# nellogrb/MultigridAnisotropicDiffusion

Measured on AMD Instinct MI355X. Metric: Mvoxel-smooths/s (and V-cycles/s) at 512^3 fp32; achieved HBM GB/s vs peak, higher is better.
Workload: dtype f32

## Files before the change

include/mad.h:

```cpp
#ifndef MAD_H
#define MAD_H

#include <stddef.h>
#include <stdint.h>

#ifdef __cplusplus
extern "C" {
#endif

#define MAD_ABI_VERSION 1

typedef enum mad_status {
  MAD_OK = 0,
  MAD_ERR_INVALID = 1,
  MAD_ERR_STATE = 2,
  MAD_ERR_DEVICE = 3,
  MAD_ERR_COMM = 4,
  MAD_ERR_SINGULAR = 5,
  MAD_ERR_UNSUPPORTED = 6,
  MAD_ERR_NOMEM = 7,
  MAD_ERR_NUMERIC = 8,
  MAD_ERR_NOT_CONVERGED = 9
} mad_status;

// ... 55 lines not shown
  uint32_t options;
  int32_t min_slab_planes;
  int32_t min_slab_voxels;
  int32_t coarse_dense_max;
  int32_t coarse_block_unknowns;
  int32_t reserved[3];
} mad_desc;

#define MAD_OPT_EAGER_RANK_VCYCLE 1u
#define MAD_OPT_OVERLAP_RANK_SWEEP 2u
#define MAD_OPT_PEER_HALO 4u
#define MAD_OPT_COARSE_NO_CHAIN 8u
#define MAD_OPT_BENCHMARK_TRACE 16u
#define MAD_OPT_NO_PLACEMENT_TUNE 32u
#define MAD_OPT_NO_RECORD_B 64u

typedef struct mad_stats {
  uint32_t steps;
  uint32_t total_cycles;
  uint32_t last_cycles;
  int32_t stalled;
  double last_relres;
  double setup_ms;
  double solve_ms;
  uint32_t num_levels;
  int32_t tensor_kind;
  int32_t colors;
  int32_t reserved[5];
} mad_stats;

// ... 10 lines not shown
int mad_set_tensor_device(mad_ctx *ctx, const void *dev_aos, int32_t dtype);
int mad_tensor_planes(const mad_ctx *ctx, int64_t *first_plane, int64_t *nplanes);
int mad_set_tensor_planes(mad_ctx *ctx, const void *host_aos, int32_t dtype,
                          int64_t first_plane, int64_t nplanes);

int mad_setup(mad_ctx *ctx);

int mad_run(mad_ctx *ctx, const void *host_in, int32_t in_dtype, void *host_out,
            int32_t out_dtype, mad_stats *stats);
int mad_run_device(mad_ctx *ctx, const void *dev_in, int32_t in_dtype, void *dev_out,
                   int32_t out_dtype, mad_stats *stats);
int mad_get_step_stats(const mad_ctx *ctx, uint32_t step, uint32_t *cycles, double *relres);
int mad_get_cycle_trace(const mad_ctx *ctx, uint32_t cap, uint32_t *step, double *relres,
                        double *seconds, uint32_t *count);
int mad_placement_trials(const mad_ctx *ctx, uint32_t cap, double *ms, uint32_t *count);

int mad_num_levels(const mad_ctx *ctx);
int mad_plan_level(const mad_desc *d, int32_t level, int64_t size[3], double spacing[3],
                   int32_t centering[3], int64_t *z_begin, int64_t *z_end,
                   int32_t *distributed);
int mad_level_info(const mad_ctx *ctx, int32_t level, int64_t size[3], double spacing[3],
                   int32_t centering[3]);

int mad_upload(mad_ctx *ctx, int32_t level, int32_t which, const double *host);
int mad_download(mad_ctx *ctx, int32_t level, int32_t which, double *host);
int mad_fill(mad_ctx *ctx, int32_t level, int32_t which, double value);
int mad_smooth(mad_ctx *ctx, int32_t level, uint32_t sweeps);
int mad_residual(mad_ctx *ctx, int32_t level, double *norm_out);
int mad_norm(mad_ctx *ctx, int32_t level, int32_t which, double *norm_out);
int mad_restrict(mad_ctx *ctx, int32_t level);
// ... 32 lines not shown
```

multigridanisotropicdiffusion_amd/_capi.py:

```python
import ctypes
import os

_HERE = os.path.dirname(os.path.abspath(__file__))
LIB_PATH = os.path.join(_HERE, "libmad_hip.so")

ABI_VERSION = 1

OK, ERR_INVALID, ERR_STATE, ERR_DEVICE, ERR_COMM, ERR_SINGULAR, ERR_UNSUPPORTED, ERR_NOMEM, \
    ERR_NUMERIC, ERR_NOT_CONVERGED = range(10)
VCYCLE, FMG, SMOOTHER = 0, 1, 2
GAUSS_SEIDEL, GAUSS_SEIDEL_LEX, WEIGHTED_JACOBI = 0, 1, 2
U8, I8, U16, I16, U32, I32, F32, F64 = range(8)
FP32, FP64, FP32_REFINE, PRECISION_AUTO = 0, 1, 2, 3
VED_HESSIAN_RECURSIVE, VED_HESSIAN_FIR = 0, 1
TENSOR_AUTO, TENSOR_ISOTROPIC, TENSOR_DIAGONAL, TENSOR_FULL = range(4)
X, B, R = 0, 1, 2
OPT_EAGER_RANK_VCYCLE = 1
OPT_OVERLAP_RANK_SWEEP = 2
OPT_PEER_HALO = 4
OPT_COARSE_NO_CHAIN = 8
OPT_BENCHMARK_TRACE = 16
OPT_NO_PLACEMENT_TUNE = 32
OPT_NO_RECORD_B = 64
VED_OPT_LINE_WALK = 1
CED_EED, CED_CED = 0, 1

EXPORTS = (
    "mad_desc_init", "mad_max_depth", "mad_create", "mad_destroy", "mad_last_error",
    "mad_get_desc", "mad_set_tensor", "mad_set_tensor_device", "mad_tensor_planes",
    "mad_set_tensor_planes", "mad_setup", "mad_run",
    "mad_run_device", "mad_get_step_stats", "mad_get_cycle_trace", "mad_placement_trials", "mad_num_levels", "mad_plan_level",
    "mad_level_info", "mad_upload",
    "mad_download", "mad_fill", "mad_smooth", "mad_residual", "mad_norm", "mad_restrict",
    "mad_residual_restrict",
    "mad_interpolate", "mad_prolongate_add", "mad_coarse_solve", "mad_vcycle", "mad_fmg",
    "mad_synchronize", "mad_bench_smooth", "mad_bench_launch_times", "mad_smooth_kernel_name", "mad_bench_vcycle", "mad_bench_synth_tensor",
    "mad_bench_synth_level", "mad_comm_unique_id", "mad_comm_init", "mad_comm_init_local", "mad_comm_init_solo",
    "mad_comm_init_rccl_solo",
    "mad_comm_selftest", "mad_slab_range", "mad_comm_allreduce_host", "mad_comm_version",
    "mad_ved_desc_init", "mad_ved_create", "mad_ved_destroy", "mad_ved_last_error",
    "mad_ved_run", "mad_ved_run_device", "mad_ved_comm_init", "mad_ved_comm_init_local",
    "mad_ved_comm_init_solo",
    "mad_ved_tensor", "mad_ved_hessian",
)

CED_EXPORTS = (
# ... 177 lines not shown
        "mad_max_depth": ([i32, i64p], i32),
        "mad_create": ([ctypes.POINTER(MadDesc), ctypes.POINTER(vp)], i32),
        "mad_destroy": ([vp], None),
        "mad_last_error": ([vp], ctypes.c_char_p),
        "mad_get_desc": ([vp, ctypes.POINTER(MadDesc)], i32),
        "mad_set_tensor": ([vp, vp, i32], i32),
        "mad_set_tensor_device": ([vp, vp, i32], i32),
        "mad_tensor_planes": ([vp, i64p, i64p], i32),
        "mad_set_tensor_planes": ([vp, vp, i32, ctypes.c_int64, ctypes.c_int64], i32),
        "mad_setup": ([vp], i32),
        "mad_run": ([vp, vp, i32, vp, i32, ctypes.POINTER(MadStats)], i32),
        "mad_run_device": ([vp, vp, i32, vp, i32, ctypes.POINTER(MadStats)], i32),
        "mad_get_step_stats": ([vp, u32, u32p, dp], i32),
        "mad_get_cycle_trace": ([vp, u32, u32p, dp, dp, u32p], i32),
        "mad_placement_trials": ([vp, u32, dp, u32p], i32),
        "mad_num_levels": ([vp], i32),
        "mad_plan_level": ([ctypes.POINTER(MadDesc), i32, i64p, dp, i32p, i64p, i64p, i32p], i32),
        "mad_level_info": ([vp, i32, i64p, dp, i32p], i32),
        "mad_upload": ([vp, i32, i32, dp], i32),
        "mad_download": ([vp, i32, i32, dp], i32),
        "mad_fill": ([vp, i32, i32, dbl], i32),
        "mad_smooth": ([vp, i32, u32], i32),
        "mad_residual": ([vp, i32, dp], i32),
        "mad_norm": ([vp, i32, i32, dp], i32),
        "mad_restrict": ([vp, i32], i32),
        "mad_residual_restrict": ([vp, i32, ctypes.POINTER(i32)], i32),
        "mad_interpolate": ([vp, i32], i32),
        "mad_prolongate_add": ([vp, i32], i32),
        "mad_coarse_solve": ([vp], i32),
        "mad_vcycle": ([vp], i32),
# ... 67 lines not shown
```

multigridanisotropicdiffusion_amd/csrc/mad_kernels.hpp:

```cpp
#pragma once
#include <hip/hip_runtime.h>

#include <climits>
#include <type_traits>
#include <cstdint>

namespace mad {

enum { KISO = 1, KDIAG = 2, KFULL = 3 };

template <int DIM, int KIND>
struct CoefLayout {
  static constexpr int NA = (KIND == KISO) ? 1 : DIM;
  static constexpr int NG = DIM;
  static constexpr int NE = (KIND == KFULL) ? DIM * (DIM - 1) / 2 : 0;
  static constexpr int N = NA + NG + NE;
};

inline int coef_count(int dim, int kind) {
  int na = (kind == KISO) ? 1 : dim;
  int ne = (kind == KFULL) ? dim * (dim - 1) / 2 : 0;
  return na + dim + ne;
}

// ... 868 lines not shown
    u_dst[e] = q < PL ? q : -1;
    u_src[e] = (uint32_t)(mirror(y0 - 1 + lj, ny) * sy + mirror(x0 - 1 + li, nx)) * TS;
  }
  const int i = x0 + tx, j = y0 + ty;
  const bool ok = i < nx && j < ny;
  const uint32_t rec_off = ok ? (uint32_t)(ty * sy + (tx & 1) * hx0 + (tx >> 1)) * (TS * RS) : 0u;
  const uint32_t pt_off = ok ? (uint32_t)(ty * sy + tx) * TS : 0u;
  const uint32_t pt_off_b = ok ? (uint32_t)(ty * sy + tx) * (uint32_t)sizeof(TB) : 0u;
  const int64_t rbase = (int64_t)y0 * sy + (x0 >> 1), pbase = (int64_t)y0 * sy + x0;
  const int il = (ty + 1) * RX + (tx + 1);
  constexpr int oyp = RX, oym = -RX;

  T up[UPT];
  T raw[RS];
  T bv = T(0);
  auto load_plane = [&](int m) {
    m = min(max(m, zlo), zhi - 1);
    const __amdgpu_buffer_rsrc_t rs = buf_rsrc(u + (int64_t)m * sz);
#pragma unroll
    for (int e = 0; e < UPT; ++e) up[e] = buf_load<T>(rs, u_src[e], 0u);
    if (ue) {
      const __amdgpu_buffer_rsrc_t re = buf_rsrc(ue + (int64_t)m * sz);
#pragma unroll
      for (int e = 0; e < UPT; ++e)
        up[e] = up[e] + (T)buf_load<TE>(re, (u_src[e] / TS) * (uint32_t)sizeof(TE), 0u);
    }
  };
  auto put_plane = [&](int m) {
    T* P = ring + (m & 3) * PL;
#pragma unroll
    for (int e = 0; e < UPT; ++e)
      if (e < UPT - 1 || u_dst[e] >= 0) P[u_dst[e]] = up[e];
  };
  auto load_pt = [&](int m) {
    m = min(max(m, 0), g.nz - 1);
    buf_load_rec<T, RS>(buf_rsrc(cf + ((int64_t)m * sz + rbase) * RS), rec_off, raw);
    if constexpr (!BREC) bv = (T)buf_load<TB>(buf_rsrc(b + (int64_t)m * sz + pbase), pt_off_b, 0u);
  };

  if (z0 - 1 >= zlo) {
// ... 166 lines not shown
    v += (T(1) - omega) * P0[0];
    load_pt(m + 1);
    if (ok) buf_store<T>(v, buf_rsrc(uo + (int64_t)m * sz + pbase), pt_off);
  }
}

template <typename T>
__global__ void __launch_bounds__(256) sumsq_k(const T* __restrict__ x, int64_t n,
                                               double* __restrict__ part) {
  double s = 0.0;
  for (int64_t q = blockIdx.x * (int64_t)blockDim.x + threadIdx.x; q < n;
       q += (int64_t)gridDim.x * blockDim.x) {
    const double v = (double)x[q];
    s += v * v;
  }
  s = block_sum<256>(s);
  if (threadIdx.x == 0) part[blockIdx.x] = s;
}

__global__ void __launch_bounds__(256) reduce_final_k(const double* __restrict__ part, int64_t n,
                                                      double* __restrict__ out) {
  double s = 0.0;
  for (int64_t q = threadIdx.x; q < n; q += blockDim.x) s += part[q];
  s = block_sum<256>(s);
  if (threadIdx.x == 0) out[0] = s;
}

template <typename W>
__device__ __forceinline__ void rtaps4(int I, int nc, int cell, int* idx, W* w) {
  const bool endv = !cell && (I == 0 || I == nc - 1);
// ... 833 lines not shown
```

multigridanisotropicdiffusion_amd/csrc/mad_solver.hip:

```cpp
#include <hip/hip_runtime.h>
#include <rocblas/rocblas.h>
#include <rocsolver/rocsolver.h>

#include <algorithm>
#include <chrono>
#include <cmath>
#include <cstdio>
#include <cstdlib>
#include <cstring>
#include <memory>
#include <mutex>
#include <stdexcept>
#include <string>
#include <thread>
#include <type_traits>
#include <vector>

#include "../../include/mad.h"
#include "mad_alloc.hpp"
#include "mad_coarse.hpp"
#include "mad_comm.hpp"
#include "mad_kernels.hpp"

using namespace mad;
// ... 197 lines not shown
  std::vector<double> step_relres;
  struct TracePoint {
    uint32_t step;
    double relres, seconds;
  };
  std::vector<TracePoint> trace;
  bool bench_trace() const { return (d.options & MAD_OPT_BENCHMARK_TRACE) != 0; }
  bool trace_active = false;
  uint32_t trace_step = 0;
  double trace_rhs = 1.0;
  std::chrono::steady_clock::time_point trace_t0{};
  void trace_push(double rr) {
    trace.push_back({trace_step, rr, std::chrono::duration<double>(std::chrono::steady_clock::now() - trace_t0).count()});
  }
  double setup_ms = 0.0;
  Comm comm;
  ~mad_ctx();
};

constexpr int TENSOR_GHOST = GHOST + 4;

struct SolverBase {
  virtual ~SolverBase() {}
  virtual void setup(mad_ctx* c) = 0;
  virtual void upload(int l, int which, const double* h) = 0;
  virtual void download(int l, int which, double* h) = 0;
  virtual void fill(int l, int which, double v) = 0;
  virtual void smooth(int l, unsigned n) = 0;
  virtual double residual(int l, bool want_norm) = 0;
  virtual double norm(int l, int which) = 0;
// ... 633 lines not shown
      REQUIRE(zr.nchunks >= 2 && zr.zc >= GHOST, MAD_ERR_UNSUPPORTED, "slab too thin for the single-launch sweep");
      *flip = 1;
      *sig = part == 3 ? L.sig : nullptr;
    } else if (part == 1) {
      zr = ZRange{0, boundary_planes(), nz - boundary_planes(), 2};
    } else if (part == 2) {
      const int ni = nz - 2 * boundary_planes();
      int chunks = std::max(1, std::min((fc.blocks + tiles - 1) / tiles, std::max(1, ni / 16)));
      const int zc = (ni + chunks - 1) / chunks;
      zr = ZRange{boundary_planes(), zc, zc, (ni + zc - 1) / zc};
    }
    return zr;
  }

  template <int KD, int TX, int TY, int NT>
  void launch_fused(LevelData<T>& L, const FusedCfg& fc, int part, bool zu = false) {
    const int ntx = (L.g.nx + TX - 1) / TX, nty = (L.g.ny + TY - 1) / TY;
    const int tiles = ntx * nty;
    int flip = 0;
    uint32_t* sig = nullptr;
    const ZRange zr = part_range(L, tiles, fc, part, &flip, &sig);
    const unsigned nb = (unsigned)(tiles * zr.nchunks);
    constexpr int NC = (KD == KFULL) ? 4 : 2;
    using FG = FusedGeom<NC, TX, TY>;
    constexpr size_t lds_u = sizeof(T) * FG::NP * FG::PLANE;
    REQUIRE(lds_u <= 160 * 1024, MAD_ERR_UNSUPPORTED,
            "fused GS tile needs " + std::to_string(lds_u) + " B of LDS (> 160 KiB)");
    constexpr size_t lds_bl = sizeof(T) * (FG::NP + NC) * FG::PLANE;
    constexpr bool bl_fits = lds_bl <= 160 * 1024;
    const bool bl = fused_b_lds(L);
    const size_t lds = bl ? lds_bl : lds_u;
    constexpr int MW = sizeof(T) == 8 ? 2 : 4;
    const PeerOut<T> po = part == 4 ? peer_out(L, buffer_index(L, L.t)) : PeerOut<T>{{nullptr, nullptr}, {nullptr, nullptr}};
    auto run = [&](auto kern) {
      {
        static std::mutex attr_mu;
        static std::vector<const void*> attr;
        std::lock_guard<std::mutex> lk(attr_mu);
        if (std::find(attr.begin(), attr.end(), (const void*)kern) == attr.end()) {
          HIP_CHECK(hipFuncSetAttribute((const void*)kern, hipFuncAttributeMaxDynamicSharedMemorySize,
                                        (int)lds));
          attr.push_back((const void*)kern);
        }
      }
      hipLaunchKernelGGL(kern, dim3(nb), dim3(NT), lds, c_->stream, L.x, L.t, L.bs ? L.bs : L.b, L.cf, L.g,
                         L.rat, zr.zc, ntx, nty, zr.zbase, zr.zstride, flip, sig, po);
    };
    if (part == 4) {
      if (L.brec)
        run(gs_fused3_k<T, KD, TX, TY, NT, MW, 2, true, true>);
      else if constexpr (bl_fits) {
        if (L.bs)
          run(gs_fused3_k<T, KD, TX, TY, NT, MW, 2, false, true, false, false, true>);
        else
          bl ? run(gs_fused3_k<T, KD, TX, TY, NT, MW, 2, false, true, true>)
             : run(gs_fused3_k<T, KD, TX, TY, NT, MW, 2, false, true>);
      } else
        run(gs_fused3_k<T, KD, TX, TY, NT, MW, 2, false, true>);
    } else if (L.brec) {
      run(gs_fused3_k<T, KD, TX, TY, NT, MW, 2, true>);
// ... 22 lines not shown
#endif
  bool fused_b_lds(const LevelData<T>& L) const {
    return MAD_FUSED_B_LDS && sizeof(T) == 4 && !L.brec && !L.bs && &L == &lv_[0];
  }

#ifndef MAD_FUSED_F32_TY
#define MAD_FUSED_F32_TY 32
#endif
  void fused_shape(const LevelData<T>& L, int* tiles, int* nchunks) const {
    const FusedCfg fc = fused_cfg();
    const int tx = 64, ty = (c_->kind == KFULL && sizeof(T) == 4) ? MAD_FUSED_F32_TY : 16;
    *tiles = ((L.g.nx + tx - 1) / tx) * ((L.g.ny + ty - 1) / ty);
    *nchunks = whole_range(L.g.nz, *tiles, fc).nchunks;
  }

  void launch_fused_part(LevelData<T>& L, int part, bool zu = false) {
    const FusedCfg fc = fused_cfg();
    if (c_->kind == KFULL) {
      if constexpr (sizeof(T) == 4)
        launch_fused<KFULL, 64, MAD_FUSED_F32_TY, MAD_FUSED_F32_TY * 32>(L, fc, part, zu);
      else
        launch_fused<KFULL, 64, 16, 512>(L, fc, part, zu);
    } else if (c_->kind == KDIAG) {
      launch_fused<KDIAG, 64, 16, 1024>(L, fc, part, zu);
    } else {
      launch_fused<KISO, 64, 16, 1024>(L, fc, part, zu);
    }
    HIP_CHECK(hipGetLastError());
  }

  std::string smooth_kernel(int l) override {
    (void)l;
    const char* tn = sizeof(T) == 4 ? "float" : "double";
    const int dim = c_->dim, kind = c_->kind;
    char buf[160];
    if (c_->d.smoother == MAD_WEIGHTED_JACOBI) {
      const LevelData<T>& L = lv_[l];
      if (dim == 3 && L.g.nx >= 16 && L.g.ny >= 16)
        std::snprintf(buf, sizeof buf, "wj3_k<%s, %d, 64, 16, %s>", tn, kind, L.brec ? "true" : "false");
      else
        std::snprintf(buf, sizeof buf, "wj_k<%s, %d, %d>", tn, dim, kind);
// ... 91 lines not shown
    if (overlap) fused_shape(L, &tiles, &nchunks);
    if (overlap && L.sig && nchunks >= 2) {
      launch_fused_part(L, 3);
      wait_all_pending();
      const uint32_t target = ++L.sig_epoch * (uint32_t)tiles;
      if (L.g.zlo_ghost)
        HIP_CHECK(hipStreamWaitValue32(c_->comm_stream, L.sig, target, hipStreamWaitValueGte, 0xFFFFFFFFu));
      if (L.g.zhi_ghost)
        HIP_CHECK(hipStreamWaitValue32(c_->comm_stream, L.sig + 1, target, hipStreamWaitValueGte,
                                       0xFFFFFFFFu));
      c_->comm.exchange_planes(L.t, L.g.sz, L.g.nz, GHOST, L.g.zlo_ghost, L.g.zhi_ghost, sizeof(T),
                               std::is_same<T, double>::value, c_->comm_stream);
      HIP_CHECK(hipEventRecord(L.ev_halo, c_->comm_stream));
    } else if (!overlap) {
      const bool zu = (zero_x0_ && &L == &lv_[0]) || L.x_zero_lazy;
      zero_x0_ = false;
      L.x_zero_lazy = false;
      launch_fused_part(L, 0, zu);
    } else {
      launch_fused_part(L, 1);
      wait_all_pending();
      HIP_CHECK(hipEventRecord(L.ev_bnd, c_->stream));
      HIP_CHECK(hipStreamWaitEvent(c_->comm_stream, L.ev_bnd, 0));
      c_->comm.exchange_planes(L.t, L.g.sz, L.g.nz, GHOST, L.g.zlo_ghost, L.g.zhi_ghost, sizeof(T),
                               std::is_same<T, double>::value, c_->comm_stream);
      HIP_CHECK(hipEventRecord(L.ev_halo, c_->comm_stream));
      launch_fused_part(L, 2);
    }
    if (e1) HIP_CHECK(hipEventRecord(e1, c_->stream));
    std::swap(L.x, L.t);
    std::swap(L.alloc[0], L.alloc[3]);
    if (overlap) {
      L.x_halo_ok = true;
// ... 134 lines not shown
    return sizeof(T) == 4 && l >= 1 && l < c_->nlev - 1 && !c_->comm.active() && !d.verbose &&
           d.iterations_per_grid >= 1 && use_fused(l) && d.gs_kernel != 4 && !lv_[l].brec &&
           c_->dim == 3;
#endif
  }
  bool zero_sweep_ok() const {
#ifdef MAD_NO_ZERO_SWEEP
    return false;
#else
    const auto& d = c_->d;
    return sizeof(T) == 4 && refine_fold_ok() && !c_->comm.active() && d.cycle == MAD_VCYCLE &&
           !d.verbose && d.iterations_per_grid >= 1 && c_->nlev > 1 && use_fused(0) && d.gs_kernel != 4 &&
           !lv_[0].brec;
#endif
  }
  double residual64(bool fold = false) {
    LevelData<T>& L = lv_[0];
    if (fold && !refine_fold_ok()) {
      hipLaunchKernelGGL((add_conv_k<T>), dim3(flat_blocks(L.g.N)), dim3(256), 0, c_->stream, u64_, L.x, L.g.N);
      HIP_CHECK(hipGetLastError());
      fold = false;
    }
    if (c_->comm.active() && c_->geom[0].distributed) {
      wait_all_pending();
      c_->comm.exchange_planes(u64_, L.g.sz, L.g.nz, 1, L.g.zlo_ghost, L.g.zhi_ghost, sizeof(double),
                               true, c_->stream);
    }
    Geo g = L.g;
    g.rs = ncoef_;
    int64_t nparts = 0;
    if (c_->dim == 3 && g.nx >= 16 && g.ny >= 16) {
      constexpr int TX = 64, TY = 16;
      const int ntx = (g.nx + TX - 1) / TX, nty = (g.ny + TY - 1) / TY;
      int chunks = std::max(1, std::min((1024 + ntx * nty - 1) / (ntx * nty), g.nz / 8));
      const int zc = (g.nz + chunks - 1) / chunks;
      chunks = (g.nz + zc - 1) / zc;
      nparts = (int64_t)ntx * nty * chunks;
      REQUIRE(nparts <= part_cap_, MAD_ERR_UNSUPPORTED, "residual partials buffer too small");
      T* const bse = (L.bs && !c_->geom[0].distributed) ? L.bs : nullptr;
      refine_emitted_bs_ = bse != nullptr;
      auto go = [&](auto K) {
        constexpr int KD = decltype(K)::value;
        auto launch = [&](auto bptr) {
          using TB = std::remove_const_t<std::remove_pointer_t<decltype(bptr)>>;
          if (fold)
            hipLaunchKernelGGL((resid3_k<double, KD, TX, TY, false, T, TB>), dim3((unsigned)nparts),
                               dim3(TX * TY), 0, c_->stream, u64_, bptr, (double*)nullptr, cf64_, g, rat64_, zc,
                               ntx, part_, L.b, (T*)nullptr, (const T*)L.x, r64_, bse);
          else
            hipLaunchKernelGGL((resid3_k<double, KD, TX, TY, false, T, TB>), dim3((unsigned)nparts),
                               dim3(TX * TY), 0, c_->stream, u64_, bptr, (double*)nullptr, cf64_, g, rat64_, zc,
                               ntx, part_, L.b, L.x, (const T*)nullptr, (double*)nullptr, bse);
        };
#ifdef MAD_NO_B32_RHS
        launch((const double*)b64_);
#else
        if (b32_exact_)
          launch((const float*)b32_);
        else
          launch((const double*)b64_);
#endif
      };
      refine_emitted_ = true;
// ... 281 lines not shown
      restrict_rhs_down(l);
      fmg_rec(l + 1);
      interpolate_up(l, false);
    }
    for (unsigned n = 0; n < c_->d.iterations_per_grid; ++n) vcycle_rec(l);
  }

  bool vgraph_ranks_ok() const {
    return !(c_->d.options & MAD_OPT_EAGER_RANK_VCYCLE) &&
           (c_->comm.mode() == Comm::RCCL || c_->comm.mode() == Comm::SOLO) && c_->d.gs_kernel != 4;
  }

  struct HaloFlags {
    bool x_ok, b_ok, brec_ok;
  };
  std::vector<HaloFlags> halo_flags() const {
    std::vector<HaloFlags> v;
    for (auto& L : lv_) v.push_back({L.x_halo_ok, L.b_halo_ok, L.brec_ok});
    return v;
  }
  void ranks_graph_entry() {
    peer_resolve_all();
    if (lv_[0].peer)
      halo(0, lv_[0].x, GHOST);
    else
      lv_[0].x_halo_ok = false;
    if (!lv_[0].brec && !lv_[0].b_halo_ok) {
      halo(0, lv_[0].b, GHOST);
      lv_[0].b_halo_ok = true;
    }
// ... 3 lines not shown
      lv_[l].b_halo_ok = lv_[l].brec_ok = false;
    }
  }

  void vcycle_fast() {
    const bool ranks = c_->comm.active();
    if (c_->d.verbose || c_->bench_trace() || vgraph_failed_ || (ranks && !vgraph_ranks_ok()) ||
        (ranks && vcycles_eager_ < 1)) {
      if (ranks) ++vcycles_eager_;
      vcycle_rec(0);
      return;
    }
    sync_brec(0);
    sync_bsplit(0);
    if (ranks) ranks_graph_entry();
    const bool zu = zero_x0_;
    if (vgraph_) {
      bool same = vgraph_ptrs_.size() == lv_.size() && vgraph_zu_ == zu;
      for (size_t l = 0; same && l < lv_.size(); ++l)
        same = vgraph_ptrs_[l].first == lv_[l].x && vgraph_ptrs_[l].second == lv_[l].t &&
               vgraph_seq_[l] == (lv_[l].peer_seq & 1);
      if (!same) {
        HIP_CHECK(hipStreamSynchronize(c_->stream));
        (void)hipGraphExecDestroy(vgraph_);
        vgraph_ = nullptr;
      }
    }
    if (!vgraph_) {
      struct Snap {
        T* x;
        T* t;
        T* a0;
        T* a3;
        bool bh;
        int seq;
      };
      auto snap = [&] {
        std::vector<Snap> v;
        for (auto& L : lv_) v.push_back({L.x, L.t, L.alloc[0], L.alloc[3], L.b_halo_ok, L.peer_seq});
        return v;
      };
      auto restore = [&](const std::vector<Snap>& v) {
        for (size_t l = 0; l < lv_.size(); ++l) {
          lv_[l].x = v[l].x;
          lv_[l].t = v[l].t;
          lv_[l].alloc[0] = v[l].a0;
          lv_[l].alloc[3] = v[l].a3;
          lv_[l].b_halo_ok = v[l].bh;
          lv_[l].peer_seq = v[l].seq;
        }
      };
      const std::vector<Snap> before = snap();
      const std::vector<HaloFlags> flags_before = halo_flags();
      hipGraph_t gph = nullptr;
      HIP_CHECK(hipStreamBeginCapture(c_->stream, hipStreamCaptureModeThreadLocal));
      bool captured = true;
      try {
        vcycle_rec(0);
        if (ranks) {
          wait_all_pending();
          peer_resolve_all();
        }
      } catch (...) {
        (void)hipStreamEndCapture(c_->stream, &gph);
        if (gph) (void)hipGraphDestroy(gph);
        gph = nullptr;
        restore(before);
        if (!ranks) throw;
        captured = false;
      }
      if (captured && hipStreamEndCapture(c_->stream, &gph) != hipSuccess) {
        gph = nullptr;
        captured = false;
      }
      const std::vector<Snap> after = snap();
      bool same = captured;
      for (size_t l = 0; same && l < before.size(); ++l)
        same = before[l].x == after[l].x && before[l].t == after[l].t &&
               ((before[l].seq ^ after[l].seq) & 1) == 0;
      vgraph_exit_flags_ = halo_flags();
      restore(before);
      if (ranks) {
        for (size_t l = 0; l < lv_.size(); ++l) {
          lv_[l].x_halo_ok = flags_before[l].x_ok;
          lv_[l].b_halo_ok = flags_before[l].b_ok;
          lv_[l].brec_ok = flags_before[l].brec_ok;
          lv_[l].x_halo_pending = false;
        }
      }
      if (same && hipGraphInstantiate(&vgraph_, gph, nullptr, nullptr, 0) != hipSuccess) {
        vgraph_ = nullptr;
        same = false;
      }
      if (gph) (void)hipGraphDestroy(gph);
      zero_x0_ = zu;
      if (!same) {
        (void)hipGetLastError();
        vgraph_failed_ = true;
        vcycle_rec(0);
        return;
      }
      vgraph_zu_ = zu;
      zero_x0_ = false;
      vgraph_ptrs_.clear();
      vgraph_seq_.clear();
      for (auto& L : lv_) {
        vgraph_ptrs_.emplace_back(L.x, L.t);
        vgraph_seq_.push_back(L.peer_seq & 1);
      }
    }
    HIP_CHECK(hipGraphLaunch(vgraph_, c_->stream));
    zero_x0_ = false;
    if (ranks) c_->comm.graph_launched(c_->stream);
    if (ranks) {
      for (size_t l = 0; l < lv_.size(); ++l) {
        lv_[l].x_halo_ok = vgraph_exit_flags_[l].x_ok;
        lv_[l].b_halo_ok = vgraph_exit_flags_[l].b_ok;
        lv_[l].brec_ok = vgraph_exit_flags_[l].brec_ok;
        lv_[l].x_halo_pending = false;
      }
    } else {
      for (size_t l = 1; l < lv_.size(); ++l) lv_[l].b_halo_ok = lv_[l].brec_ok = false;
    }
  }

  void vcycle() override { vcycle_fast(); }

  void fmg() override { fmg_rec(0); }

  void per_sweep_line(int l, int it, const char* what, bool bench) {
    if (!c_->d.verbose) {
      const double rn = residual(l, true);
      c_->trace_push(c_->trace_rhs > 0.0 ? rn / c_->trace_rhs : rn);
// ... 69 lines not shown
    unsigned total = 0;
    double relres = 0.0;
    for (unsigned step = 0; step < d.number_of_steps; ++step) {
      if (d.verbose && d.number_of_steps > 1 && c_->comm.rank() == 0)
        std::printf("\n------------ Time step n. %u / %u------------\n", step + 1, d.number_of_steps);
#ifdef MAD_NO_REFINE_FP32_PHASE
      const bool fp32_phase = false;
#else
      const bool fp32_phase = refine_ && d.cycle != MAD_SMOOTHER && d.max_cycles >= 2;
#endif
      if (bt) {
        c_->trace_t0 = std::chrono::steady_clock::now();
        c_->trace_step = step;
        c_->trace_rhs = rhs_norm();
      }
      if (refine_ && (d.cycle == MAD_FMG || fp32_phase)) to_fp32_rhs(b64_);
      if (d.cycle == MAD_FMG) {
        if (d.verbose && c_->comm.rank() == 0) std::printf("|--- Full Multigrid Cycle ---|\n");
        fmg_rec(0);
        if (refine_ && !fp32_phase) x_to_u64();
      } else if (!refine_ || fp32_phase) {
        HIP_CHECK(hipMemcpyAsync(L0.x, L0.b, sizeof(T) * N, hipMemcpyDeviceToDevice, c_->stream));
        x_changed(0);
      } else {
        HIP_CHECK(hipMemcpyAsync(u64_, b64_, sizeof(double) * N, hipMemcpyDeviceToDevice, c_->stream));
      }
      const double rhsNorm = rhs_norm();
      REQUIRE(std::isfinite(rhsNorm), MAD_ERR_NUMERIC,
              "non-finite right-hand side norm (NaN/Inf in the input image)");
      unsigned it = 0;
      std::vector<double> hist;
      const unsigned window = (d.cycle == MAD_SMOOTHER) ? 50 : 5;
      bool stalled = false;
      auto rel = [&](double resNorm) {
        REQUIRE(std::isfinite(resNorm), MAD_ERR_NUMERIC,
                "non-finite residual norm (NaN/Inf in the tensor or the iterate)");
        return (rhsNorm > 0.0) ? resNorm / rhsNorm : resNorm;
      };
      auto cycle = [&](bool zero_x0) {
        if (d.cycle == MAD_SMOOTHER) {
          smooth(0, 1);
          return;
        }
        if (d.verbose && c_->comm.rank() == 0) std::printf("\n|--- VCycle n. %u ---|\n", it + 1);
        FlagScope zu(zero_x0_, zero_x0);
        vcycle_fast();
      };
      auto record = [&](double resNorm) {
        relres = rel(resNorm);
        if (d.verbose && d.cycle == MAD_SMOOTHER && c_->comm.rank() == 0)
          std::printf("Smoother iteration n. %u: relative residual = %g\n", it + 1, relres);
        ++it;
        hist.push_back(relres);
        if (!bt || d.cycle == MAD_SMOOTHER) {
          c_->trace_step = step;
          c_->trace_push(relres);
        }
      };
      if (fp32_phase) {
        do {
          cycle(false);
          record(residual_impl(0, true, false));
          if (hist.size() >= 2 && relres > MAD_REFINE_FP32_MIN_RATE * hist[hist.size() - 2]) break;
        } while (relres > std::max(d.tolerance, MAD_REFINE_SWITCH_RELRES) && it + 1 < d.max_cycles);
        x_to_u64();
      }
      auto patch_trace = [&] {
        if (!c_->trace.empty()) c_->trace.back().relres = relres;
      };
      if (refine_) {
        relres = rel(residual64());
        if (fp32_phase) {
          hist.back() = relres;
          patch_trace();
        }
      }
      if (!fp32_phase || (relres > d.tolerance && it < d.max_cycles)) do {
        if (!refine_) {
          cycle(false);
          record(residual_impl(0, true, false));
        } else {
          if (refine_emitted_) {
            L0.b_halo_ok = false;
            L0.brec_ok = refine_emitted_bs_;
            x_changed(0);
          } else {
            to_fp32_rhs(r64_);
            fill(0, MAD_X, 0.0);
          }
          cycle(refine_emitted_ && zero_sweep_ok());
          record(residual64(true));
          if (bt && d.cycle != MAD_SMOOTHER) patch_trace();
        }
        stalled = d.stall_guard && stalled_at(hist, window, d.tolerance);
      } while (relres > d.tolerance && it < d.max_cycles && !stalled);
      stalled_any |= stalled;
      total += it;
      c_->step_cycles.push_back(it);
      c_->step_relres.push_back(relres);
      if (refine_) {
        HIP_CHECK(hipMemcpyAsync(b64_, u64_, sizeof(double) * N, hipMemcpyDeviceToDevice, c_->stream));
        b32_exact_ = false;
      } else {
        HIP_CHECK(hipMemcpyAsync(L0.b, L0.x, sizeof(T) * N, hipMemcpyDeviceToDevice, c_->stream));
        L0.b_halo_ok = L0.brec_ok = false;
      }
    }
    HIP_CHECK(hipEventRecord(e1, c_->stream));
    if (refine_ && refine_emitted_ && zero_sweep_ok()) fill(0, MAD_X, 0.0);
    void* dst = out;
    if (!dev_io) dst = scratch_bytes(N * dtype_size(out_dtype));
    if (refine_) convert_from(u64_, dst, out_dtype, N, c_->stream);
    else convert_out(L0.x, dst, out_dtype, N);
    if (!dev_io)
      HIP_CHECK(hipMemcpyAsync(out, dst, N * dtype_size(out_dtype), hipMemcpyDeviceToHost,
// ... 86 lines not shown
 private:
  mad_ctx* c_ = nullptr;
  std::vector<LevelData<T>> lv_;
  bool refine_ = false;
  double* r64alloc_[3] = {nullptr, nullptr, nullptr};
  double* u64_ = nullptr;
  double* b64_ = nullptr;
  float* b32alloc_ = nullptr;
  float* b32_ = nullptr;
  bool b32_exact_ = false;
  double* r64_ = nullptr;
  double* cf64_alloc_ = nullptr;
  double* cf64_ = nullptr;
  Rat<double> rat64_{};
  int64_t part_cap_ = 0;
  hipGraphExec_t vgraph_ = nullptr;
  bool vgraph_zu_ = false;
  std::vector<std::pair<T*, T*>> vgraph_ptrs_;
  std::vector<int> vgraph_seq_;
  bool vgraph_failed_ = false;
  uint64_t peer_timeout_ticks_ = 0;
  int peer_fallbacks_ = 0;
  std::vector<HaloFlags> vgraph_exit_flags_;
  int vcycles_eager_ = 0;
  int ncoef_ = 0;
  double* part_ = nullptr;
  double* scal_ = nullptr;
  double* hscal_ = nullptr;
  double* inv_ = nullptr;
  CoarseBlocks cblk_;
  void* scratch_ = nullptr;
  size_t scratch_cap_ = 0;
  T* gathered_ = nullptr;
  T* full_x_ = nullptr;
  int64_t gathered_cap_ = 0;
  T* cslab_ = nullptr;
  int64_t cslab_cap_ = 0;

  void release() {
    if (c_ && c_->comm_stream) (void)hipStreamSynchronize(c_->comm_stream);
    if (c_ && c_->comm.mode() != Comm::LOCAL) {
      try {
        for (size_t l = 0; l < lv_.size(); ++l)
          if (lv_[l].x_peer_pending) peer_resolve((int)l);
      } catch (...) {
      }
    }
    if (c_ && c_->stream) (void)hipStreamSynchronize(c_->stream);
    if (vgraph_) (void)hipGraphExecDestroy(vgraph_);
    vgraph_ = nullptr;
    vgraph_ptrs_.clear();
    vgraph_seq_.clear();
    vgraph_failed_ = false;
    vcycles_eager_ = 0;
    for (auto& L : lv_) {
      if (L.ev_bnd) (void)hipEventDestroy(L.ev_bnd);
      if (L.ev_halo) (void)hipEventDestroy(L.ev_halo);
      if (L.sig) (void)hipFree(L.sig);
      Comm::close_window(L.win_lo, L.win_ipc);
      Comm::close_window(L.win_hi, L.win_ipc);
      if (L.win) (void)hipFree(L.win);
      for (auto& a : L.alloc)
        if (a) (void)hipFree(a);
      if (L.cf_alloc) (void)hipFree(L.cf_alloc);
      if (L.bs_alloc) (void)hipFree(L.bs_alloc);
    }
    lv_.clear();
// ... 567 lines not shown
    }
    REQUIRE(d->size[0] * d->size[1] * (d->dim == 3 ? d->size[2] : 1) < (int64_t)INT32_MAX * 8,
            MAD_ERR_INVALID, "image too large");
    REQUIRE(d->cycle >= MAD_VCYCLE && d->cycle <= MAD_SMOOTHER, MAD_ERR_INVALID, "bad cycle");
    REQUIRE(d->smoother >= MAD_GAUSS_SEIDEL && d->smoother <= MAD_WEIGHTED_JACOBI,
            MAD_ERR_INVALID, "bad smoother");
    REQUIRE(d->precision == MAD_FP32 || d->precision == MAD_FP64 || d->precision == MAD_FP32_REFINE ||
                d->precision == MAD_PRECISION_AUTO,
            MAD_ERR_INVALID, "bad precision");
    REQUIRE(d->nranks >= 1 && d->rank >= 0 && d->rank < d->nranks, MAD_ERR_INVALID,
            "bad rank / nranks");
    REQUIRE(d->gs_kernel == 0 || d->gs_kernel == 1 || d->gs_kernel == 3 || d->gs_kernel == 4,
            MAD_ERR_INVALID, "gs_kernel must be 0, 1, 3 or 4");
    REQUIRE((d->options & ~(MAD_OPT_EAGER_RANK_VCYCLE | MAD_OPT_OVERLAP_RANK_SWEEP | MAD_OPT_PEER_HALO |
                            MAD_OPT_COARSE_NO_CHAIN | MAD_OPT_BENCHMARK_TRACE |
                            MAD_OPT_NO_PLACEMENT_TUNE | MAD_OPT_NO_RECORD_B)) == 0,
            MAD_ERR_INVALID, "unknown option bits");
    REQUIRE(d->min_slab_planes >= 0, MAD_ERR_INVALID, "min_slab_planes must be >= 0");
    REQUIRE(d->min_slab_voxels >= 0, MAD_ERR_INVALID, "min_slab_voxels must be >= 0");
    REQUIRE(d->coarse_dense_max >= 0 && d->coarse_dense_max <= MAD_COARSE_DENSE_LIMIT, MAD_ERR_INVALID,
            "coarse_dense_max must be in [0, " + std::to_string(MAD_COARSE_DENSE_LIMIT) +
                "] (a dense inverse of n unknowns takes 8 n^2 bytes on the host and twice that on the device)");
    REQUIRE(d->coarse_block_unknowns >= 0, MAD_ERR_INVALID, "coarse_block_unknowns must be >= 0");
    REQUIRE(d->tensor_kind >= MAD_TENSOR_AUTO && d->tensor_kind <= MAD_TENSOR_FULL,
            MAD_ERR_INVALID, "bad tensor kind");
    c->d = *d;
    if (c->d.precision == MAD_PRECISION_AUTO)
      c->d.precision = d->tolerance < MAD_FP32_TOLERANCE_FLOOR ? MAD_FP32_REFINE : MAD_FP32;
    if (c->d.dim == 2) c->d.size[2] = 1;
    c->dim = d->dim;
    int dev = d->device;
// ... 192 lines not shown
}

int mad_get_step_stats(const mad_ctx* c, uint32_t step, uint32_t* cycles, double* relres) {
  if (!c || step >= c->step_cycles.size()) return MAD_ERR_INVALID;
  if (cycles) *cycles = c->step_cycles[step];
  if (relres) *relres = c->step_relres[step];
  return MAD_OK;
}

int mad_placement_trials(const mad_ctx* c, uint32_t cap, double* ms, uint32_t* count) {
  if (!c || !count) return MAD_ERR_INVALID;
  const std::vector<double> v = c->solver ? c->solver->placement_ms() : std::vector<double>{};
  for (size_t q = 0; q < v.size() && q < cap; ++q)
    if (ms) ms[q] = v[q];
  *count = (uint32_t)v.size();
  return MAD_OK;
}

int mad_get_cycle_trace(const mad_ctx* c, uint32_t cap, uint32_t* step, double* relres,
                        double* seconds, uint32_t* count) {
  if (!c) return MAD_ERR_INVALID;
  const size_t n = c->trace.size();
  for (size_t q = 0; q < n && q < cap; ++q) {
    if (step) step[q] = c->trace[q].step;
    if (relres) relres[q] = c->trace[q].relres;
    if (seconds) seconds[q] = c->trace[q].seconds;
  }
  if (count) *count = (uint32_t)n;
  return MAD_OK;
}
// ... 313 lines not shown
```

multigridanisotropicdiffusion_amd/solver.py:

```python
import ctypes
import os

import numpy as np

from . import _capi as C

_DT = {np.dtype(np.uint8): C.U8, np.dtype(np.int8): C.I8, np.dtype(np.uint16): C.U16,
       np.dtype(np.int16): C.I16, np.dtype(np.uint32): C.U32, np.dtype(np.int32): C.I32,
       np.dtype(np.float32): C.F32, np.dtype(np.float64): C.F64}


def mad_dtype(dt):
    dt = np.dtype(dt)
    if dt not in _DT:
        raise TypeError(f"unsupported pixel type {dt}")
    return _DT[dt]


def max_depth(shape):
    dim = len(shape)
    n = (ctypes.c_int64 * 3)(*(list(reversed(shape)) + [1] * (3 - dim)))
    return C.load().mad_max_depth(dim, n)


# ... 238 lines not shown
        k = n.value
        st = (ctypes.c_uint32 * max(k, 1))()
        rr = (ctypes.c_double * max(k, 1))()
        sec = (ctypes.c_double * max(k, 1))()
        self._check(self._L.mad_get_cycle_trace(self._ctx, k, st, rr, sec, ctypes.byref(n)))
        return [(st[q], rr[q], sec[q]) for q in range(k)]

    def placement_trials(self):
        n = ctypes.c_uint32()
        self._check(self._L.mad_placement_trials(self._ctx, 0, None, ctypes.byref(n)))
        k = n.value
        ms = (ctypes.c_double * max(k, 1))()
        self._check(self._L.mad_placement_trials(self._ctx, k, ms, ctypes.byref(n)))
        return [ms[q] for q in range(k)]

    @property
    def resolved_precision(self):
        d = C.MadDesc()
        self._check(self._L.mad_get_desc(self._ctx, ctypes.byref(d)))
        return d.precision

    def bench_smooth(self, level, sweeps):
        t, k, n = ctypes.c_double(), ctypes.c_double(), ctypes.c_uint32()
        self._check(self._L.mad_bench_smooth(self._ctx, level, sweeps, ctypes.byref(t),
                                             ctypes.byref(k), ctypes.byref(n)))
        return t.value, k.value, n.value

    def bench_launch_times(self):
        buf = (ctypes.c_float * 4096)()
        n = ctypes.c_uint32()
# ... 25 lines not shown
```

Baseline: 120,900.

## Fuse per-step RHS passes and start first sweep directly from the RHS

Adds a step_begin kernel that computes the RHS norm while copying the source into b and the reordered bs buffer in one pass. This replaces the separate conversion, copy and norm passes. The first V-cycle's fused sweep now reads the initial iterate straight from b, so the x=b memcpy is skipped. Separate V-cycle graphs are cached per start form (plain, zero, rhs), and in refine mode the u64/b64 copy between steps becomes a pointer swap with a folded fp64 residual. This saves several full-grid HBM passes per time step, at the cost of more graph variants, more state flags, and new correctness risk in the buffer handling.

```diff
diff --git a/include/mad.h b/include/mad.h
--- a/include/mad.h
+++ b/include/mad.h
@@ -93,6 +93,7 @@
 #define MAD_OPT_BENCHMARK_TRACE 16u
 #define MAD_OPT_NO_PLACEMENT_TUNE 32u
 #define MAD_OPT_NO_RECORD_B 64u
+#define MAD_OPT_PLAIN_STEP_PASSES 128u
 
 typedef struct mad_stats {
   uint32_t steps;
@@ -133,6 +134,7 @@
 int mad_get_cycle_trace(const mad_ctx *ctx, uint32_t cap, uint32_t *step, double *relres,
                         double *seconds, uint32_t *count);
 int mad_placement_trials(const mad_ctx *ctx, uint32_t cap, double *ms, uint32_t *count);
+int mad_vcycle_captures(const mad_ctx *ctx, uint32_t *count);
 
 int mad_num_levels(const mad_ctx *ctx);
 int mad_plan_level(const mad_desc *d, int32_t level, int64_t size[3], double spacing[3],
diff --git a/multigridanisotropicdiffusion_amd/_capi.py b/multigridanisotropicdiffusion_amd/_capi.py
--- a/multigridanisotropicdiffusion_amd/_capi.py
+++ b/multigridanisotropicdiffusion_amd/_capi.py
@@ -22,6 +22,7 @@
 OPT_BENCHMARK_TRACE = 16
 OPT_NO_PLACEMENT_TUNE = 32
 OPT_NO_RECORD_B = 64
+OPT_PLAIN_STEP_PASSES = 128
 VED_OPT_LINE_WALK = 1
 CED_EED, CED_CED = 0, 1
 
@@ -29,7 +30,7 @@
     "mad_desc_init", "mad_max_depth", "mad_create", "mad_destroy", "mad_last_error",
     "mad_get_desc", "mad_set_tensor", "mad_set_tensor_device", "mad_tensor_planes",
     "mad_set_tensor_planes", "mad_setup", "mad_run",
-    "mad_run_device", "mad_get_step_stats", "mad_get_cycle_trace", "mad_placement_trials", "mad_num_levels", "mad_plan_level",
+    "mad_run_device", "mad_get_step_stats", "mad_get_cycle_trace", "mad_placement_trials", "mad_vcycle_captures", "mad_num_levels", "mad_plan_level",
     "mad_level_info", "mad_upload",
     "mad_download", "mad_fill", "mad_smooth", "mad_residual", "mad_norm", "mad_restrict",
     "mad_residual_restrict",
@@ -237,6 +238,7 @@
         "mad_get_step_stats": ([vp, u32, u32p, dp], i32),
         "mad_get_cycle_trace": ([vp, u32, u32p, dp, dp, u32p], i32),
         "mad_placement_trials": ([vp, u32, dp, u32p], i32),
+        "mad_vcycle_captures": ([vp, u32p], i32),
         "mad_num_levels": ([vp], i32),
         "mad_plan_level": ([ctypes.POINTER(MadDesc), i32, i64p, dp, i32p, i64p, i64p, i32p], i32),
         "mad_level_info": ([vp, i32, i64p, dp, i32p], i32),
diff --git a/multigridanisotropicdiffusion_amd/csrc/mad_kernels.hpp b/multigridanisotropicdiffusion_amd/csrc/mad_kernels.hpp
--- a/multigridanisotropicdiffusion_amd/csrc/mad_kernels.hpp
+++ b/multigridanisotropicdiffusion_amd/csrc/mad_kernels.hpp
@@ -906,16 +906,21 @@
   T up[UPT];
   T raw[RS];
   T bv = T(0);
+  const bool has_u = std::is_same<T, TE>::value || u != nullptr;
   auto load_plane = [&](int m) {
     m = min(max(m, zlo), zhi - 1);
-    const __amdgpu_buffer_rsrc_t rs = buf_rsrc(u + (int64_t)m * sz);
-#pragma unroll
-    for (int e = 0; e < UPT; ++e) up[e] = buf_load<T>(rs, u_src[e], 0u);
+    if (has_u) {
+      const __amdgpu_buffer_rsrc_t rs = buf_rsrc(u + (int64_t)m * sz);
+#pragma unroll
+      for (int e = 0; e < UPT; ++e) up[e] = buf_load<T>(rs, u_src[e], 0u);
+    }
     if (ue) {
       const __amdgpu_buffer_rsrc_t re = buf_rsrc(ue + (int64_t)m * sz);
 #pragma unroll
-      for (int e = 0; e < UPT; ++e)
-        up[e] = up[e] + (T)buf_load<TE>(re, (u_src[e] / TS) * (uint32_t)sizeof(TE), 0u);
+      for (int e = 0; e < UPT; ++e) {
+        const T ev = (T)buf_load<TE>(re, (u_src[e] / TS) * (uint32_t)sizeof(TE), 0u);
+        up[e] = has_u ? up[e] + ev : ev;
+      }
     }
   };
   auto put_plane = [&](int m) {
@@ -1112,6 +1117,47 @@
     const double v = (double)x[q];
     s += v * v;
   }
+  s = block_sum<256>(s);
+  if (threadIdx.x == 0) part[blockIdx.x] = s;
+}
+
+template <typename S, typename T>
+__global__ void __launch_bounds__(256) step_begin_k(const S* __restrict__ src, T* __restrict__ b,
+                                                    T* __restrict__ bs, Geo g, int64_t n,
+                                                    double* __restrict__ part) {
+  const int64_t stride = (int64_t)gridDim.x * blockDim.x;
+  int64_t q = blockIdx.x * (int64_t)blockDim.x + threadIdx.x;
+  const int nx = g.nx, ny = g.ny;
+  const int64_t srem = stride % g.sz;
+  const int dk = (int)(stride / g.sz), dj = (int)(srem / nx), di = (int)(srem % nx);
+  const int64_t qrem = q % g.sz;
+  int k = (int)(q / g.sz), j = (int)(qrem / nx), i = (int)(qrem % nx);
+  double s = 0.0;
+  auto take = [&](S sv, int64_t p) {
+    const double v = (double)sv;
+    s += v * v;
+    if (b) b[p] = (T)sv;
+    if (bs) bs[cidx(g, i, j, k)] = (T)sv;
+    i += di;
+    if (i >= nx) {
+      i -= nx;
+      ++j;
+    }
+    j += dj;
+    if (j >= ny) {
+      j -= ny;
+      ++k;
+    }
+    k += dk;
+  };
+  for (; q + 3 * stride < n; q += 4 * stride) {
+    S sv[4];
+#pragma unroll
+    for (int e = 0; e < 4; ++e) sv[e] = src[q + e * stride];
+#pragma unroll
+    for (int e = 0; e < 4; ++e) take(sv[e], q + e * stride);
+  }
+  for (; q < n; q += stride) take(src[q], q);
   s = block_sum<256>(s);
   if (threadIdx.x == 0) part[blockIdx.x] = s;
 }
diff --git a/multigridanisotropicdiffusion_amd/csrc/mad_solver.hip b/multigridanisotropicdiffusion_amd/csrc/mad_solver.hip
--- a/multigridanisotropicdiffusion_amd/csrc/mad_solver.hip
+++ b/multigridanisotropicdiffusion_amd/csrc/mad_solver.hip
@@ -235,6 +235,8 @@
     trace.push_back({trace_step, rr, std::chrono::duration<double>(std::chrono::steady_clock::now() - trace_t0).count()});
   }
   double setup_ms = 0.0;
+  uint32_t vcycle_captures = 0;
+  bool plain_step_passes() const { return (d.options & MAD_OPT_PLAIN_STEP_PASSES) != 0; }
   Comm comm;
   ~mad_ctx();
 };
@@ -898,7 +900,7 @@
   }
 
   template <int KD, int TX, int TY, int NT>
-  void launch_fused(LevelData<T>& L, const FusedCfg& fc, int part, bool zu = false) {
+  void launch_fused(LevelData<T>& L, const FusedCfg& fc, int part, bool zu = false, const T* uin = nullptr) {
     const int ntx = (L.g.nx + TX - 1) / TX, nty = (L.g.ny + TY - 1) / TY;
     const int tiles = ntx * nty;
     int flip = 0;
@@ -927,7 +929,7 @@
           attr.push_back((const void*)kern);
         }
       }
-      hipLaunchKernelGGL(kern, dim3(nb), dim3(NT), lds, c_->stream, L.x, L.t, L.bs ? L.bs : L.b, L.cf, L.g,
+      hipLaunchKernelGGL(kern, dim3(nb), dim3(NT), lds, c_->stream, uin ? uin : L.x, L.t, L.bs ? L.bs : L.b, L.cf, L.g,
                          L.rat, zr.zc, ntx, nty, zr.zbase, zr.zstride, flip, sig, po);
     };
     if (part == 4) {
@@ -980,17 +982,17 @@
     *nchunks = whole_range(L.g.nz, *tiles, fc).nchunks;
   }
 
-  void launch_fused_part(LevelData<T>& L, int part, bool zu = false) {
+  void launch_fused_part(LevelData<T>& L, int part, bool zu = false, const T* uin = nullptr) {
     const FusedCfg fc = fused_cfg();
     if (c_->kind == KFULL) {
       if constexpr (sizeof(T) == 4)
-        launch_fused<KFULL, 64, MAD_FUSED_F32_TY, MAD_FUSED_F32_TY * 32>(L, fc, part, zu);
+        launch_fused<KFULL, 64, MAD_FUSED_F32_TY, MAD_FUSED_F32_TY * 32>(L, fc, part, zu, uin);
       else
-        launch_fused<KFULL, 64, 16, 512>(L, fc, part, zu);
+        launch_fused<KFULL, 64, 16, 512>(L, fc, part, zu, uin);
     } else if (c_->kind == KDIAG) {
-      launch_fused<KDIAG, 64, 16, 1024>(L, fc, part, zu);
+      launch_fused<KDIAG, 64, 16, 1024>(L, fc, part, zu, uin);
     } else {
-      launch_fused<KISO, 64, 16, 1024>(L, fc, part, zu);
+      launch_fused<KISO, 64, 16, 1024>(L, fc, part, zu, uin);
     }
     HIP_CHECK(hipGetLastError());
   }
@@ -1112,9 +1114,11 @@
       HIP_CHECK(hipEventRecord(L.ev_halo, c_->comm_stream));
     } else if (!overlap) {
       const bool zu = (zero_x0_ && &L == &lv_[0]) || L.x_zero_lazy;
-      zero_x0_ = false;
+      const T* const uin = (rhs_x0_ && &L == &lv_[0]) ? L.b : nullptr;
+      REQUIRE(!(zu && uin), MAD_ERR_STATE, "zero-iterate and rhs-iterate sweep at once");
+      zero_x0_ = rhs_x0_ = false;
       L.x_zero_lazy = false;
-      launch_fused_part(L, 0, zu);
+      launch_fused_part(L, 0, zu, uin);
     } else {
       launch_fused_part(L, 1);
       wait_all_pending();
@@ -1279,8 +1283,31 @@
            !lv_[0].brec;
 #endif
   }
-  double residual64(bool fold = false) {
+  bool rhs_x0_ = false;
+  bool rhs_sweep_ok() const {
+    const auto& d = c_->d;
+    return !c_->plain_step_passes() && c_->dim == 3 && !c_->comm.active() && d.cycle == MAD_VCYCLE &&
+           !d.verbose && !c_->bench_trace() && d.iterations_per_grid >= 1 && c_->nlev > 1 && use_fused(0) &&
+           d.gs_kernel != 4;
+  }
+  bool step_begin_ok() const { return !c_->plain_step_passes() && lv_[0].bs && !c_->comm.active(); }
+  template <typename S>
+  double step_begin(const S* src) {
     LevelData<T>& L = lv_[0];
+    const int64_t n = L.g.N;
+    const unsigned nb = flat_blocks(n, 2048);
+    T* const bout = (const void*)src == (const void*)L.b ? nullptr : L.b;
+    T* const bsout = (use_fused(0) || c_->d.cycle == MAD_VCYCLE) ? L.bs : nullptr;
+    hipLaunchKernelGGL((step_begin_k<S, T>), dim3(nb), dim3(256), 0, c_->stream, src, bout, bsout, L.g, n, part_);
+    HIP_CHECK(hipGetLastError());
+    L.b_halo_ok = false;
+    L.brec_ok = bsout != nullptr;
+    return std::sqrt(finish_norm2(nb, false));
+  }
+
+  double residual64(bool fold = false, bool from_x = false) {
+    LevelData<T>& L = lv_[0];
+    REQUIRE(!from_x || (fold && refine_fold_ok()), MAD_ERR_STATE, "fp64 residual of x without the folded pass");
     if (fold && !refine_fold_ok()) {
       hipLaunchKernelGGL((add_conv_k<T>), dim3(flat_blocks(L.g.N)), dim3(256), 0, c_->stream, u64_, L.x, L.g.N);
       HIP_CHECK(hipGetLastError());
@@ -1310,8 +1337,9 @@
           using TB = std::remove_const_t<std::remove_pointer_t<decltype(bptr)>>;
           if (fold)
             hipLaunchKernelGGL((resid3_k<double, KD, TX, TY, false, T, TB>), dim3((unsigned)nparts),
-                               dim3(TX * TY), 0, c_->stream, u64_, bptr, (double*)nullptr, cf64_, g, rat64_, zc,
-                               ntx, part_, L.b, (T*)nullptr, (const T*)L.x, r64_, bse);
+                               dim3(TX * TY), 0, c_->stream, from_x ? (const double*)nullptr : u64_, bptr,
+                               (double*)nullptr, cf64_, g, rat64_, zc, ntx, part_, L.b, (T*)nullptr,
+                               (const T*)L.x, r64_, bse);
           else
             hipLaunchKernelGGL((resid3_k<double, KD, TX, TY, false, T, TB>), dim3((unsigned)nparts),
                                dim3(TX * TY), 0, c_->stream, u64_, bptr, (double*)nullptr, cf64_, g, rat64_, zc,
@@ -1623,6 +1651,20 @@
   struct HaloFlags {
     bool x_ok, b_ok, brec_ok;
   };
+  enum { VG_PLAIN = 0, VG_ZERO = 1, VG_RHS = 2, VG_FORMS = 3 };
+  struct VGraph {
+    hipGraphExec_t exec = nullptr;
+    int form = VG_PLAIN;
+    std::vector<std::pair<T*, T*>> ptrs;
+    std::vector<int> seq;
+    std::vector<HaloFlags> exit_flags;
+  };
+  void drop_vgraphs() {
+    for (auto& v : vg_) {
+      if (v.exec) (void)hipGraphExecDestroy(v.exec);
+      v = VGraph{};
+    }
+  }
   std::vector<HaloFlags> halo_flags() const {
     std::vector<HaloFlags> v;
     for (auto& L : lv_) v.push_back({L.x_halo_ok, L.b_halo_ok, L.brec_ok});
@@ -1656,19 +1698,21 @@
     sync_brec(0);
     sync_bsplit(0);
     if (ranks) ranks_graph_entry();
-    const bool zu = zero_x0_;
-    if (vgraph_) {
-      bool same = vgraph_ptrs_.size() == lv_.size() && vgraph_zu_ == zu;
+    const bool zu = zero_x0_, bx = rhs_x0_;
+    const int form = zu ? VG_ZERO : (bx ? VG_RHS : VG_PLAIN);
+    VGraph& vg = vg_[c_->plain_step_passes() ? 0 : form];
+    if (vg.exec) {
+      bool same = vg.ptrs.size() == lv_.size() && vg.form == form;
       for (size_t l = 0; same && l < lv_.size(); ++l)
-        same = vgraph_ptrs_[l].first == lv_[l].x && vgraph_ptrs_[l].second == lv_[l].t &&
-               vgraph_seq_[l] == (lv_[l].peer_seq & 1);
+        same = vg.ptrs[l].first == lv_[l].x && vg.ptrs[l].second == lv_[l].t &&
+               vg.seq[l] == (lv_[l].peer_seq & 1);
       if (!same) {
         HIP_CHECK(hipStreamSynchronize(c_->stream));
-        (void)hipGraphExecDestroy(vgraph_);
-        vgraph_ = nullptr;
-      }
-    }
-    if (!vgraph_) {
+        (void)hipGraphExecDestroy(vg.exec);
+        vg.exec = nullptr;
+      }
+    }
+    if (!vg.exec) {
       struct Snap {
         T* x;
         T* t;
@@ -1696,6 +1740,7 @@
       const std::vector<HaloFlags> flags_before = halo_flags();
       hipGraph_t gph = nullptr;
       HIP_CHECK(hipStreamBeginCapture(c_->stream, hipStreamCaptureModeThreadLocal));
+      ++c_->vcycle_captures;
       bool captured = true;
       try {
         vcycle_rec(0);
@@ -1720,7 +1765,7 @@
       for (size_t l = 0; same && l < before.size(); ++l)
         same = before[l].x == after[l].x && before[l].t == after[l].t &&
                ((before[l].seq ^ after[l].seq) & 1) == 0;
-      vgraph_exit_flags_ = halo_flags();
+      vg.exit_flags = halo_flags();
       restore(before);
       if (ranks) {
         for (size_t l = 0; l < lv_.size(); ++l) {
@@ -1730,35 +1775,36 @@
           lv_[l].x_halo_pending = false;
         }
       }
-      if (same && hipGraphInstantiate(&vgraph_, gph, nullptr, nullptr, 0) != hipSuccess) {
-        vgraph_ = nullptr;
+      if (same && hipGraphInstantiate(&vg.exec, gph, nullptr, nullptr, 0) != hipSuccess) {
+        vg.exec = nullptr;
         same = false;
       }
       if (gph) (void)hipGraphDestroy(gph);
       zero_x0_ = zu;
+      rhs_x0_ = bx;
       if (!same) {
         (void)hipGetLastError();
         vgraph_failed_ = true;
         vcycle_rec(0);
         return;
       }
-      vgraph_zu_ = zu;
-      zero_x0_ = false;
-      vgraph_ptrs_.clear();
-      vgraph_seq_.clear();
+      vg.form = form;
+      zero_x0_ = rhs_x0_ = false;
+      vg.ptrs.clear();
+      vg.seq.clear();
       for (auto& L : lv_) {
-        vgraph_ptrs_.emplace_back(L.x, L.t);
-        vgraph_seq_.push_back(L.peer_seq & 1);
-      }
-    }
-    HIP_CHECK(hipGraphLaunch(vgraph_, c_->stream));
-    zero_x0_ = false;
+        vg.ptrs.emplace_back(L.x, L.t);
+        vg.seq.push_back(L.peer_seq & 1);
+      }
+    }
+    HIP_CHECK(hipGraphLaunch(vg.exec, c_->stream));
+    zero_x0_ = rhs_x0_ = false;
     if (ranks) c_->comm.graph_launched(c_->stream);
     if (ranks) {
       for (size_t l = 0; l < lv_.size(); ++l) {
-        lv_[l].x_halo_ok = vgraph_exit_flags_[l].x_ok;
-        lv_[l].b_halo_ok = vgraph_exit_flags_[l].b_ok;
-        lv_[l].brec_ok = vgraph_exit_flags_[l].brec_ok;
+        lv_[l].x_halo_ok = vg.exit_flags[l].x_ok;
+        lv_[l].b_halo_ok = vg.exit_flags[l].b_ok;
+        lv_[l].brec_ok = vg.exit_flags[l].brec_ok;
         lv_[l].x_halo_pending = false;
       }
     } else {
@@ -1858,18 +1904,35 @@
         c_->trace_step = step;
         c_->trace_rhs = rhs_norm();
       }
-      if (refine_ && (d.cycle == MAD_FMG || fp32_phase)) to_fp32_rhs(b64_);
+      const bool fp32_start = !refine_ || d.cycle == MAD_FMG || fp32_phase;
+      const bool one_pass = fp32_start && step_begin_ok();
+      double rhsNorm = 0.0;
+      if (one_pass) {
+        if (!refine_)
+          rhsNorm = step_begin((const T*)L0.b);
+        else if (b32_exact_)
+          rhsNorm = step_begin((const float*)b32_);
+        else
+          rhsNorm = step_begin((const double*)b64_);
+      } else if (refine_ && fp32_start) {
+        to_fp32_rhs(b64_);
+      }
+      bool first_from_b = false;
       if (d.cycle == MAD_FMG) {
         if (d.verbose && c_->comm.rank() == 0) std::printf("|--- Full Multigrid Cycle ---|\n");
         fmg_rec(0);
         if (refine_ && !fp32_phase) x_to_u64();
       } else if (!refine_ || fp32_phase) {
-        HIP_CHECK(hipMemcpyAsync(L0.x, L0.b, sizeof(T) * N, hipMemcpyDeviceToDevice, c_->stream));
-        x_changed(0);
+        if (rhs_sweep_ok()) {
+          first_from_b = true;
+        } else {
+          HIP_CHECK(hipMemcpyAsync(L0.x, L0.b, sizeof(T) * N, hipMemcpyDeviceToDevice, c_->stream));
+          x_changed(0);
+        }
       } else {
         HIP_CHECK(hipMemcpyAsync(u64_, b64_, sizeof(double) * N, hipMemcpyDeviceToDevice, c_->stream));
       }
-      const double rhsNorm = rhs_norm();
+      if (!one_pass) rhsNorm = rhs_norm();
       REQUIRE(std::isfinite(rhsNorm), MAD_ERR_NUMERIC,
               "non-finite right-hand side norm (NaN/Inf in the input image)");
       unsigned it = 0;
@@ -1888,6 +1951,8 @@
         }
         if (d.verbose && c_->comm.rank() == 0) std::printf("\n|--- VCycle n. %u ---|\n", it + 1);
         FlagScope zu(zero_x0_, zero_x0);
+        FlagScope bx(rhs_x0_, first_from_b);
+        first_from_b = false;
         vcycle_fast();
       };
       auto record = [&](double resNorm) {
@@ -1901,19 +1966,20 @@
           c_->trace_push(relres);
         }
       };
+      const bool switch_fold = fp32_phase && !c_->plain_step_passes() && refine_fold_ok();
       if (fp32_phase) {
         do {
           cycle(false);
           record(residual_impl(0, true, false));
           if (hist.size() >= 2 && relres > MAD_REFINE_FP32_MIN_RATE * hist[hist.size() - 2]) break;
         } while (relres > std::max(d.tolerance, MAD_REFINE_SWITCH_RELRES) && it + 1 < d.max_cycles);
-        x_to_u64();
+        if (!switch_fold) x_to_u64();
       }
       auto patch_trace = [&] {
         if (!c_->trace.empty()) c_->trace.back().relres = relres;
       };
       if (refine_) {
-        relres = rel(residual64());
+        relres = rel(switch_fold ? residual64(true, true) : residual64());
         if (fp32_phase) {
           hist.back() = relres;
           patch_trace();
@@ -1942,7 +2008,12 @@
       total += it;
       c_->step_cycles.push_back(it);
       c_->step_relres.push_back(relres);
-      if (refine_) {
+      if (refine_ && !c_->plain_step_passes()) {
+        if (step + 1 < d.number_of_steps) {
+          std::swap(u64_, b64_);
+          b32_exact_ = false;
+        }
+      } else if (refine_) {
         HIP_CHECK(hipMemcpyAsync(b64_, u64_, sizeof(double) * N, hipMemcpyDeviceToDevice, c_->stream));
         b32_exact_ = false;
       } else {
@@ -2059,14 +2130,10 @@
   double* cf64_ = nullptr;
   Rat<double> rat64_{};
   int64_t part_cap_ = 0;
-  hipGraphExec_t vgraph_ = nullptr;
-  bool vgraph_zu_ = false;
-  std::vector<std::pair<T*, T*>> vgraph_ptrs_;
-  std::vector<int> vgraph_seq_;
+  VGraph vg_[VG_FORMS];
   bool vgraph_failed_ = false;
   uint64_t peer_timeout_ticks_ = 0;
   int peer_fallbacks_ = 0;
-  std::vector<HaloFlags> vgraph_exit_flags_;
   int vcycles_eager_ = 0;
   int ncoef_ = 0;
   double* part_ = nullptr;
@@ -2092,10 +2159,7 @@
       }
     }
     if (c_ && c_->stream) (void)hipStreamSynchronize(c_->stream);
-    if (vgraph_) (void)hipGraphExecDestroy(vgraph_);
-    vgraph_ = nullptr;
-    vgraph_ptrs_.clear();
-    vgraph_seq_.clear();
+    drop_vgraphs();
     vgraph_failed_ = false;
     vcycles_eager_ = 0;
     for (auto& L : lv_) {
@@ -2693,7 +2757,8 @@
             MAD_ERR_INVALID, "gs_kernel must be 0, 1, 3 or 4");
     REQUIRE((d->options & ~(MAD_OPT_EAGER_RANK_VCYCLE | MAD_OPT_OVERLAP_RANK_SWEEP | MAD_OPT_PEER_HALO |
                             MAD_OPT_COARSE_NO_CHAIN | MAD_OPT_BENCHMARK_TRACE |
-                            MAD_OPT_NO_PLACEMENT_TUNE | MAD_OPT_NO_RECORD_B)) == 0,
+                            MAD_OPT_NO_PLACEMENT_TUNE | MAD_OPT_NO_RECORD_B |
+                            MAD_OPT_PLAIN_STEP_PASSES)) == 0,
             MAD_ERR_INVALID, "unknown option bits");
     REQUIRE(d->min_slab_planes >= 0, MAD_ERR_INVALID, "min_slab_planes must be >= 0");
     REQUIRE(d->min_slab_voxels >= 0, MAD_ERR_INVALID, "min_slab_voxels must be >= 0");
@@ -2916,6 +2981,12 @@
   for (size_t q = 0; q < v.size() && q < cap; ++q)
     if (ms) ms[q] = v[q];
   *count = (uint32_t)v.size();
+  return MAD_OK;
+}
+
+int mad_vcycle_captures(const mad_ctx* c, uint32_t* count) {
+  if (!c || !count) return MAD_ERR_INVALID;
+  *count = c->vcycle_captures;
   return MAD_OK;
 }
 
diff --git a/multigridanisotropicdiffusion_amd/solver.py b/multigridanisotropicdiffusion_amd/solver.py
--- a/multigridanisotropicdiffusion_amd/solver.py
+++ b/multigridanisotropicdiffusion_amd/solver.py
@@ -276,6 +276,11 @@
         self._check(self._L.mad_placement_trials(self._ctx, k, ms, ctypes.byref(n)))
         return [ms[q] for q in range(k)]
 
+    def vcycle_captures(self):
+        n = ctypes.c_uint32()
+        self._check(self._L.mad_vcycle_captures(self._ctx, ctypes.byref(n)))
+        return n.value
+
     @property
     def resolved_precision(self):
         d = C.MadDesc()
```

Measured after the change: 118,200. -2.3%, worse.
